# software-mansion/smelter

Measured on AMD Instinct MI355X. Metric: composited frames/sec, 8x1080p->1 4K scene, higher is better.
Workload: dtype u8 (f32 colour conversion: the WGSL sequence value for value; Lanczos on f16-pair MFMA with f32 accumulate, f16 resampler intermediate); 1 GPU; configs[2]: 8x1080p YUV420 inputs tiled -> 3840x2160 YUV420, Tiles + Rescaler(border_radius 24) + text label per tile, GpuOptimized (linear-light Lanczos3 + blend); inputs=8, layouts=33, prime_frames=4676, input_ring=12, frames_in_flight=2, parallelism=single GPU

## Files before the change

### smelter_amd/csrc/smr_fused.hip

```cpp
#include "smr_fused_compose.h"
#include "smr_fused_ingest.h"
#include "smr_ingest_wave.h"

#include <cstdlib>

namespace {

bool fused_disabled(smr_ctx *ctx) {
#ifdef SMR_LAB
    if (!ctx->ablate_read) {
        const char *a = getenv("SMR_ABLATE");
        ctx->ablate = a ? atoi(a) : 0;
        ctx->ablate_read = true;
    }
#endif
    return ctx->fused_disabled == 1;
}

bool frame_is_opaque(u32 fmt) { return frame_format_is_opaque_ycbcr(fmt); }

constexpr size_t SLOT_TARGET = SMR_SLOT_TARGET, SLOT_INGEST_NODE = SMR_SLOT_INGEST_NODE, SLOT_NODE0 = SMR_SLOT_NODE0, SLOT_TILE0 = SMR_SLOT_TILE0,
                 SLOT_TRANSPOSED0 = SMR_SLOT_TRANSPOSED0, SLOT_TRANSPOSED_SINGLE = SMR_SLOT_TRANSPOSED_SINGLE, SLOT_REDUCED0 = SMR_SLOT_REDUCED0;

bool rgb12_node_serves(smr_ctx *ctx, const smr_frame *f, const smr_resample_plan &plan, const smr_surface *tile) {
// ... 485 lines not shown
    }
    if (!wjobs_f16_alpha.empty()) {
        rc = launch_wave(ctx, wjobs_f16_alpha, nullptr, true, true, false, true);
        if (rc != SMR_OK) return rc;
    }
    if (!wjobs_sa_rgba_alpha.empty()) {
        rc = launch_wave(ctx, wjobs_sa_rgba_alpha, nullptr, true, false, true, true);
        if (rc != SMR_OK) return rc;
    }
    if (!wjobs_sa.empty()) {
        rc = launch_wave(ctx, wjobs_sa, nullptr, false, false, true);
        if (rc != SMR_OK) return rc;
    }
    if (!wjobs_sa_rgba.empty()) {
        rc = launch_wave(ctx, wjobs_sa_rgba, nullptr, true, false, true);
        if (rc != SMR_OK) return rc;
    }
    for (const MTransposeBack &b : transposed) {
        rc = launch_transpose<u32>(ctx, b.tile_t, b.tile);
        if (rc != SMR_OK) return rc;
    }
    if (!jobs.empty()) {
        rc = launch_ingest(ctx, jobs);
        if (rc != SMR_OK) return rc;
    }

    if (fuse_out) {
        StageScope scope(ctx, SMR_STAGE_FUSED_COMPOSE);
        ctx->kernel_launches[SMR_KERNEL_COMPOSE_OUTPUT]++;
        u32 n_banded = cm->count_known ? *cm->h_count : n_first * (u32)B_AREA_BANDS;
        if (n_banded > b_tiles * (u32)B_AREA_BANDS) n_banded = b_tiles * (u32)B_AREA_BANDS;
        if (ctx->debug_ingest)
            fprintf(stderr, "k_compose_output: %u tiles, %u bands on the list (%s; predicted tiles %u, last read back %u)\n", b_tiles, n_banded, cm->count_known ? "known" : "predicted", n_first, *cm->h_count);
        dim3 grid(n_banded + (b_tiles + B_COPY_TILES - 1) / B_COPY_TILES, 1, 1);
        const TileList *full = (const TileList *)cm->d_list;
        const TileClass *tc = (const TileClass *)cm->d_class;
        const int flags = (ctx->srgb() ? 1 : 0) | ((ctx->ablate >> 8) << 8);
        SurfView p0, p1, p2;
        int nv;
        if (fuse_rgba) {
            p0 = p1 = p2 = view_of(rgba_target);
            nv = 2;
        } else {
            p0 = view_of(out->planes[0]); p1 = view_of(out->planes[1]);
            nv = out->format == SMR_FRAME_NV12 ? 1 : 0;
            p2 = nv ? p1 : view_of(out->planes[2]);
        }
        typedef void (*ComposeKernel)(SurfView, SurfView, SurfView, int, int, const DevLayout *, const DevMask *, int, int, int, const float *, int, int,
                                      const TileClass *, const TileList *, int, int);
        static const ComposeKernel kernels[3][2] = {{k_compose_output<0, false>, k_compose_output<0, true>},
                                                    {k_compose_output<1, false>, k_compose_output<1, true>},
                                                    {k_compose_output<2, false>, k_compose_output<2, true>}};
        hipLaunchKernelGGL(kernels[nv][big_list ? 1 : 0], grid, dim3(256), 0, ctx->stream, p0, p1, p2, (int)out_w, (int)out_h, packed.layouts, packed.masks,
                           packed.n, packed.n_masks, flags, ctx->d_tables, (int)b_tiles_x, (int)b_tiles, tc, full, (int)n_banded, cm->counter);
        SMR_HIP(ctx, hipGetLastError());
        rc = smr_pack_done(ctx, &packed);
        if (rc != SMR_OK) return rc;
        if (fuse_rgba && out) return smr_rgba_to_frame(ctx, rgba_target, out);
        return SMR_OK;
    }

    smr_surface *target = out_rgba ? out_rgba : smr_cached_surface(ctx, SLOT_TARGET, out_w, out_h, SMR_PX_RGBA8);
    if (!target) return SMR_ERR_OOM;
    rc = smr_launch_apply_layouts(ctx, target, &packed);
    if (rc != SMR_OK) return rc;
    rc = smr_pack_done(ctx, &packed);
    if (rc != SMR_OK) return rc;
// ... 201 lines not shown
```

### smelter_amd/csrc/smr_fused_compose.h

```cpp
#pragma once

#include <type_traits>

#include "smr_convert_dev.h"
#include "smr_layout_dev.h"

namespace {

__device__ __forceinline__ u32 b_off(int row, u32 pitch, int col_bytes) { return (u32)__umul24((u32)row, pitch) + (u32)col_bytes; }

constexpr int B_TILE_W = 128, B_TILE_H = 16;
constexpr int B_MAX_LAYOUTS = 48;
constexpr int B_MAX_MASKS = 96;
static_assert(sizeof(DevLayout) % 16 == 0 && sizeof(DevMask) % 16 == 0, "LDS copies move 16 B words");

#ifndef SMR_COMPOSE_MIN_WAVES
#define SMR_COMPOSE_MIN_WAVES 6
#endif
constexpr int B_MIN_WAVES = SMR_COMPOSE_MIN_WAVES;
constexpr int B_BAND_ROWS = SMR_COMPOSE_BAND_ROWS;
static_assert(B_TILE_H % B_BAND_ROWS == 0 && B_BAND_ROWS >= 2, "a band fits the LDS pixel state");

inline u32 compose_predict(const PackedLayouts &p, int tiles_x, int tiles_y, std::vector<u32> &bitmap) {
    const int tiles = tiles_x * tiles_y, words = (tiles + 31) / 32;
    bitmap.assign((size_t)words, 0u);
    auto mark = [&](float x0, float y0, float x1, float y1) {
        int tx0 = (int)floorf(x0 / (float)B_TILE_W), tx1 = (int)floorf(x1 / (float)B_TILE_W);
        int ty0 = (int)floorf(y0 / (float)B_TILE_H), ty1 = (int)floorf(y1 / (float)B_TILE_H);
        tx0 = tx0 < 0 ? 0 : tx0; ty0 = ty0 < 0 ? 0 : ty0;
        tx1 = tx1 >= tiles_x ? tiles_x - 1 : tx1; ty1 = ty1 >= tiles_y ? tiles_y - 1 : ty1;
        for (int ty = ty0; ty <= ty1; ty++)
            for (int tx = tx0; tx <= tx1; tx++) {
                const int t = ty * tiles_x + tx;
                bitmap[t >> 5] |= 1u << (t & 31);
            }
    };
    auto corners = [&](float left, float top, float w, float h, float c, const DevLayout &L) {
        if (!(c > 0.0f)) return;
        const float bx0 = (float)L.bx0, by0 = (float)L.by0, bx1 = (float)L.bx1 - 1.0f, by1 = (float)L.by1 - 1.0f;
        const float xs[2][2] = {{left, left + c}, {left + w - c, left + w}}, ys[2][2] = {{top, top + c}, {top + h - c, top + h}};
// ... 209 lines not shown
    o.w = div_cr((float)a, 255.0f, 1.0f / 255.0f);
    return o;
}

__device__ __forceinline__ u32 aligned_texel(const DevLayout &L, int px, int py) {
    return g_ld_u32(L.src.ptr + b_off(clampi(py - L.iy, 0, L.tex_h - 1), L.src.pitch, clampi(px - L.ix, 0, L.tex_w - 1) * 4));
}

__device__ __forceinline__ u32 compose_px(u32 a, const DevLayout &L, const DevMask *__restrict__ masks, int px, int py, bool is_base,
                                          u32 raw_pre, int srgb, const float *__restrict__ dec, const float *__restrict__ thr) {
    float fx, fy, lx, ly;
    if (!layout_covers(L, px, py, fx, fy, lx, ly)) return a;
    const bool solid = is_base || layout_solid_box(L, masks, fx, fy, fx, fy);
    if (L.type != 0) {
        if (solid && (L.flags & DL_COLOR_OPAQUE)) return L.solid_px;
        const float4 frag = solid ? make_float4(L.color[0], L.color[1], L.color[2], L.color[3])
                                  : layout_fragment(L, masks, fx, fy, lx, ly, make_float4(0.f, 0.f, 0.f, 0.f));
        return blend_store(a, frag, srgb, dec, thr);
    }
    const bool aligned = (L.flags & DL_ALIGNED) && L.src_kind != 0;
    u32 raw = 0u;
    float4 sample;
    if (aligned) {
        raw = raw_pre;
        sample = decode_texel(raw, srgb, dec);
    } else {
        sample = layout_texture_sample(L, px, py, lx, ly, srgb, dec);
    }
    const float4 frag = solid ? sample : layout_fragment(L, masks, fx, fy, lx, ly, sample);
    if (aligned && (raw >> 24) == 255u && frag.x == sample.x && frag.y == sample.y && frag.z == sample.z && frag.w == sample.w) return raw;
    return blend_store(a, frag, srgb, dec, thr);
}

template <int NV>
__device__ __forceinline__ void store_yuv_block(const u32 (&acc)[8], int px0, int py0, int W, const SurfView &yp, const SurfView &up, const SurfView &vp) {
    const bool half = px0 + 3 >= W;
    if (NV == 2) {
        u8 *o = yp.ptr + b_off(py0, yp.pitch, px0 * 4);
        if (half) {
            *(uint2 *)o = make_uint2(acc[0], acc[1]);
            *(uint2 *)(o + yp.pitch) = make_uint2(acc[4], acc[5]);
        } else {
            *(uint4 *)o = make_uint4(acc[0], acc[1], acc[2], acc[3]);
            *(uint4 *)(o + yp.pitch) = make_uint4(acc[4], acc[5], acc[6], acc[7]);
        }
        return;
    }
    float cr[8], cg[8], cb[8];
#pragma unroll
    for (int k = 0; k < 8; k++) {
        cr[k] = (float)(acc[k] & 0xffu);
        cg[k] = (float)((acc[k] >> 8) & 0xffu);
        cb[k] = (float)((acc[k] >> 16) & 0xffu);
    }
    u32 yrow0 = 0, yrow1 = 0;
#pragma unroll
    for (int k = 0; k < 4; k++) {
        yrow0 |= yuv_luma_byte(acc[k], cr[k], cg[k], cb[k]) << (8 * k);
        yrow1 |= yuv_luma_byte(acc[4 + k], cr[4 + k], cg[4 + k], cb[4 + k]) << (8 * k);
    }
    if (half) {
        *(u16 *)(yp.ptr + b_off(py0, yp.pitch, px0)) = (u16)yrow0;
        *(u16 *)(yp.ptr + b_off(py0 + 1, yp.pitch, px0)) = (u16)yrow1;
    } else {
        *(u32 *)(yp.ptr + b_off(py0, yp.pitch, px0)) = yrow0;
        *(u32 *)(yp.ptr + b_off(py0 + 1, yp.pitch, px0)) = yrow1;
    }
    u32 uv[2][2];
#pragma unroll
    for (int j = 0; j < 2; j++) {
        const int a = 2 * j, b = 2 * j + 1, c = 4 + 2 * j, d = 4 + 2 * j + 1;
        const u32 q = yuv_chroma_bytes(acc[a], acc[b], acc[c], acc[d], (cr[a] + cr[b]) + (cr[c] + cr[d]), (cg[a] + cg[b]) + (cg[c] + cg[d]),
                                       (cb[a] + cb[b]) + (cb[c] + cb[d]));
        uv[j][0] = q & 0xffu;
        uv[j][1] = q >> 8;
    }
    const int cx = px0 >> 1, cy = py0 >> 1;
    if (NV == 0) {
        if (half) {
            up.ptr[b_off(cy, up.pitch, cx)] = (u8)uv[0][0];
            vp.ptr[b_off(cy, vp.pitch, cx)] = (u8)uv[0][1];
        } else {
            *(u16 *)(up.ptr + b_off(cy, up.pitch, cx)) = (u16)(uv[0][0] | (uv[1][0] << 8));
            *(u16 *)(vp.ptr + b_off(cy, vp.pitch, cx)) = (u16)(uv[0][1] | (uv[1][1] << 8));
        }
    } else if (half) {
        *(u16 *)(up.ptr + b_off(cy, up.pitch, cx * 2)) = (u16)(uv[0][0] | (uv[0][1] << 8));
    } else {
        *(u32 *)(up.ptr + b_off(cy, up.pitch, cx * 2)) = uv[0][0] | (uv[0][1] << 8) | (uv[1][0] << 16) | (uv[1][1] << 24);
    }
}

__device__ __forceinline__ u32 list_slot(u32 *count, bool want) {
#ifdef SMR_EMU
    return want ? atomicAdd(count, 1u) : 0u;
#else
    const unsigned long long m = __ballot(want);
    if (m == 0ull) return 0u;
    const u32 rank = __builtin_amdgcn_mbcnt_hi((u32)(m >> 32), __builtin_amdgcn_mbcnt_lo((u32)m, 0u));
    u32 base = 0u;
    if (want && rank == 0u) base = atomicAdd(count, (u32)__popcll(m));
    return (u32)__builtin_amdgcn_readlane((int)base, (int)__builtin_ctzll(m)) + rank;
#endif
}
__device__ __forceinline__ bool wave_any(bool v) {
#ifdef SMR_EMU
    return true;
#else
    return __ballot(v) != 0ull;
#endif
}

template <int NV, bool BIG>
__device__ __forceinline__ void compose_full(const TileFull *__restrict__ pre, int band, int rh, const SurfView &yp, const SurfView &up, const SurfView &vp, int W, int H,
                                             const DevLayout *__restrict__ layouts_g, const DevMask *__restrict__ masks_g, int n, int n_masks,
                                             int srgb_and_ablate, const float *__restrict__ tables, int tiles_x, float *s_tab) {
    const int tile = (int)pre->tile;
    constexpr int BAND_PX = B_TILE_W * B_BAND_ROWS;
    constexpr int SWEEPS = 2;
    static_assert(BAND_PX % 512 == 0 && BAND_PX <= 2048, "whole slabs; a list entry keeps the pixel's index in IDX_BITS bits");
    constexpr int IDX_BITS = BIG ? 11 : (BAND_PX <= 1024 ? 10 : 11);
    constexpr bool WIDE = BIG || ((B_MAX_LAYOUTS + 1) > (1 << (16 - IDX_BITS)));
    typedef typename std::conditional<WIDE, u32, u16>::type entry_t;
    __shared__ u32 s_touch[MAX_LAYOUT_WORDS];
    __shared__ u32 s_px[BAND_PX];
    __shared__ entry_t s_list[BAND_PX];
    __shared__ u32 s_count;
    __shared__ __attribute__((aligned(16))) DevLayout s_lay[B_MAX_LAYOUTS];
    __shared__ __attribute__((aligned(16))) DevMask s_mask[B_MAX_MASKS];
    const int tid = threadIdx.x;
    u32 acc[8] = {0u, 0u, 0u, 0u, 0u, 0u, 0u, 0u};
    const int tile_y = tile / tiles_x;
    const int tx0 = (tile - tile_y * tiles_x) * B_TILE_W, ty0 = tile_y * B_TILE_H + band;
    const int px0 = tx0 + 4 * (tid & 31), py0 = ty0 + 2 * (tid >> 5);
    __syncthreads();
    {
        static_assert(SMR_TABLE_FLOATS % 4 == 0 && SMR_TABLE_FLOATS / 4 <= 256, "one 16 B word of the tables per thread");
        constexpr int LW = (B_MAX_LAYOUTS * (int)(sizeof(DevLayout) / 16) + 255) / 256, MW = (B_MAX_MASKS * (int)(sizeof(DevMask) / 16) + 255) / 256;
        const uint4 *gl = (const uint4 *)layouts_g, *gm = (const uint4 *)masks_g, *gt = (const uint4 *)tables;
        const int nl = BIG ? 0 : n * (int)(sizeof(DevLayout) / 16), nm = BIG ? 0 : n_masks * (int)(sizeof(DevMask) / 16);
        uint4 wl[LW], wm[MW], wt = make_uint4(0u, 0u, 0u, 0u);
#pragma unroll
        for (int k = 0; k < LW; k++) {
            wl[k] = wt;
            if (tid + 256 * k < nl) wl[k] = gl[tid + 256 * k];
        }
#pragma unroll
        for (int k = 0; k < MW; k++) {
            wm[k] = wt;
            if (tid + 256 * k < nm) wm[k] = gm[tid + 256 * k];
        }
        if (tid < SMR_TABLE_FLOATS / 4) wt = gt[tid];
        u32 touch_w = 0u;
        if (tid < MAX_LAYOUT_WORDS) touch_w = pre->touch[tid];
#pragma unroll
        for (int k = 0; k < LW; k++)
            if (tid + 256 * k < nl) ((uint4 *)s_lay)[tid + 256 * k] = wl[k];
#pragma unroll
        for (int k = 0; k < MW; k++)
            if (tid + 256 * k < nm) ((uint4 *)s_mask)[tid + 256 * k] = wm[k];
        if (tid < SMR_TABLE_FLOATS / 4) ((uint4 *)s_tab)[tid] = wt;
        if (tid < MAX_LAYOUT_WORDS) s_touch[tid] = touch_w;
        if (tid == 0) s_count = 0u;
// ... 107 lines not shown
    }
    }
    __syncthreads();

    const u32 total = s_count;
#pragma unroll 1
    for (u32 k0 = 0; k0 < total; k0 += 256u) {
        const bool act = k0 + (u32)tid < total;
        const u32 e = act ? (u32)s_list[k0 + tid] : 0u;
        const int idx = (int)(e & ((1u << IDX_BITS) - 1u)), from = (int)(e >> IDX_BITS) - 1;
        const int px = tx0 + (idx & (B_TILE_W - 1)), py = ty0 + (idx >> 7);
        u32 a = s_px[idx];
        for (int wi = start < 0 ? 0 : (start >> 5); wi < words; wi++) {
            u32 bits = __builtin_amdgcn_readfirstlane(s_touch[wi]);
            if (start >= 0 && wi == (start >> 5)) bits &= ~((2u << (start & 31)) - 1u);
            while (bits) {
                const int li = (wi << 5) + __builtin_ctz(bits);
                bits &= bits - 1;
                const DevLayout *Lp = &layouts[li];
                const int bx0 = __builtin_amdgcn_readfirstlane(Lp->bx0), bx1 = __builtin_amdgcn_readfirstlane(Lp->bx1);
                const int by0 = __builtin_amdgcn_readfirstlane(Lp->by0), by1 = __builtin_amdgcn_readfirstlane(Lp->by1);
                const bool need = act && li > from && px >= bx0 && px < bx1 && py >= by0 && py < by1;
                if (!wave_any(need)) continue;
                const DevLayout L = load_uniform(Lp);
                u32 raw = 0u;
                if (need && L.type == 0 && (L.flags & DL_ALIGNED) && L.src_kind != 0) raw = aligned_texel(L, px, py);
                if (need) a = compose_px(a, L, masks, px, py, false, raw, srgb, dec, thr);
            }
        }
        if (act) s_px[idx] = a;
    }
    __syncthreads();
    if (!no_block) {
        const int lx0 = px0 - tx0, ly0 = py0 - ty0;
        const uint4 t0 = *(const uint4 *)&s_px[ly0 * B_TILE_W + lx0], t1 = *(const uint4 *)&s_px[(ly0 + 1) * B_TILE_W + lx0];
        acc[0] = t0.x; acc[1] = t0.y; acc[2] = t0.z; acc[3] = t0.w;
        acc[4] = t1.x; acc[5] = t1.y; acc[6] = t1.z; acc[7] = t1.w;
        store_yuv_block<NV>(acc, px0, py0, W, yp, up, vp);
    }
}

#ifndef SMR_COPY_TILES
#define SMR_COPY_TILES 1
#endif
constexpr int B_COPY_TILES = SMR_COPY_TILES;
static_assert(B_COPY_TILES == 1 || B_COPY_TILES == 2, "one or two tiles per workgroup");

template <int NV, bool BIG>
__global__ __launch_bounds__(256, B_MIN_WAVES) void k_compose_output(SurfView yp, SurfView up, SurfView vp, int W, int H,
                                                        const DevLayout *__restrict__ layouts_g, const DevMask *__restrict__ masks_g,
                                                        int n, int n_masks, int srgb_and_ablate, const float *__restrict__ tables,
                                                        int tiles_x, int tiles, const TileClass *__restrict__ tc, const TileList *__restrict__ full,
                                                        int n_banded, int counter) {
    const int tid = threadIdx.x;
#if defined(SMR_PRIO_COMPOSE) && !defined(SMR_EMU)
    __builtin_amdgcn_s_setprio(SMR_PRIO_COMPOSE);
#endif
    __shared__ __attribute__((aligned(16))) float s_tab[SMR_TABLE_FLOATS];
    const int rest = (int)blockIdx.x - n_banded;
    const TileFull *full_entry = nullptr, *full_entry2 = nullptr;
    int full_entries = 1, full_entries2 = 1;
    if (rest < 0) {
        if (blockIdx.x >= full->count[counter]) return;
        full_entry = &full->e[blockIdx.x];
    } else {
    const int t0 = rest * B_COPY_TILES;
    const int bx = 4 * (tid & 31), by = 2 * (tid >> 5);
    TileClass c[B_COPY_TILES];
#pragma unroll
    for (int k = 0; k < B_COPY_TILES; k++) {
        c[k] = tc[min(t0 + k, tiles - 1)];
        if (t0 + k >= tiles) c[k].kind = TC_SKIP;
    }
    u32 acc[B_COPY_TILES][8];
    bool on[B_COPY_TILES];
    bool aligned = true;
#pragma unroll
    for (int k = 0; k < B_COPY_TILES; k++) {
        const int tile = t0 + k, ty = tile / tiles_x;
        on[k] = c[k].kind <= TC_TEXTURE && !((srgb_and_ablate >> 8) & 64) && (tile - ty * tiles_x) * B_TILE_W + bx < W && ty * B_TILE_H + by < H;
        if (c[k].kind == TC_TEXTURE && ((((uintptr_t)c[k].base) & 15) != 0 || (c[k].pitch_or_px & 15) != 0)) aligned = false;
        if ((W & 3) && (tile - ty * tiles_x) * B_TILE_W + B_TILE_W > W) aligned = false;
    }
    if (aligned) {
        uint4 ra[B_COPY_TILES], rb[B_COPY_TILES];
#pragma unroll
        for (int k = 0; k < B_COPY_TILES; k++) {
            const bool tex = on[k] && c[k].kind == TC_TEXTURE;
            const u8 *r0 = tex ? c[k].base + b_off(by, c[k].pitch_or_px, bx * 4) : (const u8 *)tables;
            const u8 *r1 = tex ? r0 + c[k].pitch_or_px : (const u8 *)tables;
            ra[k] = g_ld_u32x4(r0);
            rb[k] = g_ld_u32x4(r1);
        }
#pragma unroll
        for (int k = 0; k < B_COPY_TILES; k++) {
            const bool tex = c[k].kind == TC_TEXTURE;
            const u32 fill = c[k].kind == TC_COLOUR ? c[k].pitch_or_px : 0u;
            acc[k][0] = tex ? ra[k].x : fill; acc[k][1] = tex ? ra[k].y : fill; acc[k][2] = tex ? ra[k].z : fill; acc[k][3] = tex ? ra[k].w : fill;
            acc[k][4] = tex ? rb[k].x : fill; acc[k][5] = tex ? rb[k].y : fill; acc[k][6] = tex ? rb[k].z : fill; acc[k][7] = tex ? rb[k].w : fill;
        }
    } else {
#pragma unroll
        for (int k = 0; k < B_COPY_TILES; k++) {
            const u32 fill = c[k].kind == TC_COLOUR ? c[k].pitch_or_px : 0u;
#pragma unroll
            for (int q = 0; q < 8; q++) acc[k][q] = fill;
            if (on[k] && c[k].kind == TC_TEXTURE) {
                const u8 *r0 = c[k].base + b_off(by, c[k].pitch_or_px, bx * 4), *r1 = r0 + c[k].pitch_or_px;
                const int tile = t0 + k, cols = W - ((tile - (tile / tiles_x) * tiles_x) * B_TILE_W + bx);
#pragma unroll
                for (int q = 0; q < 4; q++)
                    if (q < cols) { acc[k][q] = g_ld_u32(r0 + 4 * q); acc[k][4 + q] = g_ld_u32(r1 + 4 * q); }
            }
        }
    }
#pragma unroll
    for (int k = 0; k < B_COPY_TILES; k++) {
        const int tile = t0 + k, ty = tile / tiles_x;
        if (on[k]) store_yuv_block<NV>(acc[k], (tile - ty * tiles_x) * B_TILE_W + bx, ty * B_TILE_H + by, W, yp, up, vp);
    }
#pragma unroll 1
    for (int k = 0; k < B_COPY_TILES; k++) {
        if (c[k].kind != TC_SAMPLED || ((srgb_and_ablate >> 8) & 32)) continue;
        __syncthreads();
        for (int i = tid; i < SMR_TABLE_FLOATS; i += 256) s_tab[i] = tables[i];
        __syncthreads();
        const DevLayout L = load_uniform(&layouts_g[c[k].pitch_or_px]);
        const int tile = t0 + k, ty = tile / tiles_x;
        const int px0 = (tile - ty * tiles_x) * B_TILE_W + bx, py0 = ty * B_TILE_H + by;
        if (px0 < W && py0 < H) {
            u32 a[8];
            composite_sampled_opaque_block(L, px0, py0, srgb_and_ablate & 1, s_tab, s_tab + 256, a);
            store_yuv_block<NV>(a, px0, py0, W, yp, up, vp);
        }
    }
#pragma unroll 1
    for (int k = 0; k < B_COPY_TILES; k++) {
        if (c[k].kind != TC_SELECT) continue;
        const int tile = t0 + k, ty = tile / tiles_x;
        const int px0 = (tile - ty * tiles_x) * B_TILE_W + bx, py0 = ty * B_TILE_H + by;
        u32 a[8] = {0u, 0u, 0u, 0u, 0u, 0u, 0u, 0u};
        u32 open_px = 0xffu;
#pragma unroll 1
        for (int q = 0; q < 4; q++) {
            const u32 li = (c[k].pitch_or_px >> (8 * q)) & 0xffu;
            if (li == 0xffu) break;
            const DevLayout &L = layouts_g[li];
            const int lx0 = L.bx0, ly0 = L.by0, lx1 = L.bx1, ly1 = L.by1;
            const bool colour = L.type != 0;
            const u32 solid = L.solid_px;
#pragma unroll
            for (int i = 0; i < 8; i++) {
                const int px = px0 + (i & 3), py = py0 + (i >> 2);
                if (((open_px >> i) & 1u) && px >= lx0 && px < lx1 && py >= ly0 && py < ly1) {
                    a[i] = colour ? solid : aligned_texel(L, px, py);
                    open_px &= ~(1u << i);
                }
            }
        }
        if (px0 < W && py0 < H) store_yuv_block<NV>(a, px0, py0, W, yp, up, vp);
    }
    if (c[0].kind == TC_FULL && (int)c[0].pitch_or_px + (int)(uintptr_t)c[0].base > n_banded) {
        full_entry = &full->e[c[0].pitch_or_px];
        full_entries = (int)(uintptr_t)c[0].base;
    }
    if (B_COPY_TILES > 1 && c[B_COPY_TILES - 1].kind == TC_FULL && (int)c[B_COPY_TILES - 1].pitch_or_px + (int)(uintptr_t)c[B_COPY_TILES - 1].base > n_banded) {
        const TileFull *e = &full->e[c[B_COPY_TILES - 1].pitch_or_px];
        if (full_entry) { full_entry2 = e; full_entries2 = (int)(uintptr_t)c[B_COPY_TILES - 1].base; }
        else { full_entry = e; full_entries = (int)(uintptr_t)c[B_COPY_TILES - 1].base; }
    }
    }
#ifdef SMR_COMPOSE_NO_FULL
    if (full_entry || full_entry2) return;
#endif
#pragma unroll 1
    for (int q = 0; q < 2; q++) {
        const TileFull *e = q == 0 ? full_entry : full_entry2;
        if (!e) break;
        const int entries = q == 0 ? full_entries : full_entries2;
#pragma unroll 1
        for (int j = 0; j < entries; j++) {
            if (rest >= 0 && (int)(e - full->e) + j < n_banded) continue;
            const u32 bw = __builtin_amdgcn_readfirstlane(e[j].band);
            compose_full<NV, BIG>(&e[j], (int)(bw & 0xffu), (int)(bw >> 8), yp, up, vp, W, H, layouts_g, masks_g, n, n_masks, srgb_and_ablate, tables, tiles_x, s_tab);
        }
    }
}

}
```

### smelter_amd/csrc/smr_ingest_common.h

```cpp
#pragma once

#include "smr_convert_dev.h"
#include "smr_resample_dev.h"

typedef _Float16 f16x8 __attribute__((ext_vector_type(8)));
typedef float f32x4 __attribute__((ext_vector_type(4)));

#ifdef SMR_EMU
#include "emu_device.h"
#else
#define dev_perm(hi, lo, sel) __builtin_amdgcn_perm((hi), (lo), (sel))
#define dev_alignbyte(hi, lo, sh) __builtin_amdgcn_alignbyte((hi), (lo), (sh))
#define dev_udot4(a, b, c) __builtin_amdgcn_udot4((a), (b), (c), false)
#define dev_fmed3(a, b, c) __builtin_amdgcn_fmed3f((a), (b), (c))
#define dev_mad24(a, b, c) ((u32)__umul24((a), (b)) + (c))
#define dev_readfirstlane(x) __builtin_amdgcn_readfirstlane(x)
#define dev_mfma_16x16x32_f16(a, b, c) __builtin_amdgcn_mfma_f32_16x16x32_f16((a), (b), (c), 0, 0, 0)
#define dev_wait_vmcnt0() __builtin_amdgcn_s_waitcnt(0x0f70)
#define dev_mov_dpp_quad_swap(x) __builtin_amdgcn_mov_dpp((x), 0xb1, 0xf, 0xf, true)
#define dev_sched_barrier() __builtin_amdgcn_sched_barrier(0)
#define dev_wave_lds_sync() __builtin_amdgcn_wave_barrier()
__device__ __forceinline__ u32 dev_lds_u32(u32 byte_offset) {
    typedef __attribute__((address_space(3))) const u32 lds_u32;
    return *(lds_u32 *)(uintptr_t)byte_offset;
}
#endif

namespace {

struct MConv {
    float ky, krv, kgu, kgv, kbu, cr, cg, cb, ylo, yhi, clo, chi;
};

constexpr int M_LUT_ENTRIES = 768;

struct MDirect {
    const u8 *cls;
    int tiles_x, nv;
    SurfView yp, up, vp;
};

inline MConv m_conv_constants(bool full) {
    const double ys = full ? 1.0 : 255.0 / 219.0, y0 = full ? 0.0 : 16.0;
    const double cs = full ? 1.0 / 16.0 : 255.0 / (16.0 * 224.0);
    const double c0 = full ? 0.0 : 16.0 * 16.0, half = full ? 16.0 * 127.5 : 16.0 * 112.0;
    MConv K;
    K.ky = (float)ys;
    K.krv = (float)(1.5748 * cs); K.kgu = (float)(-0.1873 * cs); K.kgv = (float)(-0.4681 * cs); K.kbu = (float)(1.8556 * cs);
    const double bias = 1024.0 + 256.0 + 0.5;
    K.cr = (float)(bias - ys * y0 - 1.5748 * cs * (c0 + half));
    K.cg = (float)(bias - ys * y0 + (0.1873 + 0.4681) * cs * (c0 + half));
    K.cb = (float)(bias - ys * y0 - 1.8556 * cs * (c0 + half));
// ... 79 lines not shown
```

### smelter_amd/csrc/smr_internal.h

```cpp
#pragma once


#include <hip/hip_runtime.h>
#include <hip/hip_fp16.h>

#include <cstdarg>
#include <cstdint>
#include <cstdio>
#include <cstring>
#include <string>
#include <vector>

#include "smr.h"

constexpr int SMR_INGEST_LAB_FUSED = 5;
#ifdef SMR_LAB
constexpr bool SMR_LAB_BUILD = true;
#else
constexpr bool SMR_LAB_BUILD = false;
#endif

#ifndef SMR_COMPOSE_BAND_ROWS
#define SMR_COMPOSE_BAND_ROWS 8
#endif
// ... 5 lines not shown
#define SMR_ENC_ENTRIES 1664
#define SMR_LUT16_WORDS (256 + SMR_ENC_ENTRIES)

#define SMR_NUM_STAGES 8
enum {
    SMR_STAGE_INGEST = 0,
    SMR_STAGE_RESAMPLE = 1,
    SMR_STAGE_LAYOUT = 2,
    SMR_STAGE_OUTPUT = 3,
    SMR_STAGE_FUSED_INGEST = 4,
    SMR_STAGE_FUSED_COMPOSE = 5,
};

constexpr size_t SMR_SURFACE_TAIL = 16;

struct smr_surface {
    void *ptr = nullptr;
    size_t pitch = 0;
    u32 w = 0, h = 0, fmt = 0;
    bool owned = false;
    size_t capacity = 0;

};

#if defined(__HIPCC__) && !defined(SMR_EMU)
typedef u32 g_u32x2 __attribute__((ext_vector_type(2)));
typedef u32 g_u32x3 __attribute__((ext_vector_type(3)));
typedef u32 g_u32x4 __attribute__((ext_vector_type(4)));
#define SMR_GLOBAL_PTR(T, p) ((__attribute__((address_space(1))) T *)(uintptr_t)(p))
__device__ __forceinline__ u32 g_ld_u32(const void *p) { return *SMR_GLOBAL_PTR(const u32, p); }
__device__ __forceinline__ uint2 g_ld_u32x2(const void *p) { const g_u32x2 v = *SMR_GLOBAL_PTR(const g_u32x2, p); return make_uint2(v.x, v.y); }
__device__ __forceinline__ uint4 g_ld_u32x4(const void *p) { const g_u32x4 v = *SMR_GLOBAL_PTR(const g_u32x4, p); return make_uint4(v.x, v.y, v.z, v.w); }
__device__ __forceinline__ void g_st_u32(void *p, u32 v) { *SMR_GLOBAL_PTR(u32, p) = v; }
__device__ __forceinline__ void g_st_u32x3(void *p, u32 a, u32 b, u32 c) { g_u32x3 v; v.x = a; v.y = b; v.z = c; *SMR_GLOBAL_PTR(g_u32x3, p) = v; }
__device__ __forceinline__ void g_st_u32x4(void *p, uint4 q) { g_u32x4 v; v.x = q.x; v.y = q.y; v.z = q.z; v.w = q.w; *SMR_GLOBAL_PTR(g_u32x4, p) = v; }
typedef int g_i32x2 __attribute__((ext_vector_type(2)));
__device__ __forceinline__ int2 g_ld_uniform_i32x2(const void *p) { const g_i32x2 v = *((__attribute__((address_space(4))) const g_i32x2 *)(uintptr_t)(p)); return make_int2(v.x, v.y); }
#define SMR_KEEP_SCALAR(x) asm volatile("" : "+s"(x))
#else
static inline u32 g_ld_u32(const void *p) { return *(const u32 *)p; }
static inline uint2 g_ld_u32x2(const void *p) { return *(const uint2 *)p; }
static inline uint4 g_ld_u32x4(const void *p) { return *(const uint4 *)p; }
static inline void g_st_u32(void *p, u32 v) { *(u32 *)p = v; }
static inline void g_st_u32x3(void *p, u32 a, u32 b, u32 c) { ((u32 *)p)[0] = a; ((u32 *)p)[1] = b; ((u32 *)p)[2] = c; }
static inline void g_st_u32x4(void *p, uint4 q) { *(uint4 *)p = q; }
static inline int2 g_ld_uniform_i32x2(const void *p) { return *(const int2 *)p; }
#define SMR_KEEP_SCALAR(x) do { } while (0)
#endif

struct LayoutSlot {
    void *host = nullptr;
    void *dev = nullptr;
    size_t bytes = 0;
    hipEvent_t done = nullptr;
    bool busy = false;
    bool unfenced = false;
    size_t resident_bytes = 0;
    uint64_t last_reuse = 0;
};

struct StagePending {
    hipEvent_t a, b;
    int stage;
};

struct TileClassMap {
    std::vector<uint8_t> key;
    bool ready = false;
    void *d_class = nullptr;
    uint8_t *d_direct = nullptr;
    void *d_list = nullptr;
    size_t n = 0;
    uint32_t *h_count = nullptr;
    hipEvent_t count_ev = nullptr;
    bool count_pending = false, count_known = false;
    uint64_t class_serial = 0, count_serial = 0;
// ... 188 lines not shown
```

Before: 19900 frames/s.

## Pair YUV stores across lanes, fast colour path with repair, multi-tile copy runs

Converts RGB to YUV with a fast yuvfast path and recomputes exactly only when a flag marks a byte as uncertain. Adjacent lanes trade rows and chroma through DPP quad swaps, so each lane issues one wider 8-byte luma store and one 4-byte chroma store instead of several narrow ones. Copy workgroups now walk a short run of tiles, prefetching the next tile's texels while storing the current one, which halves the copy grid. The cost is more per-lane control flow, an extra branch on the repair path, and a deferred pass for sampled, select and full tiles.

```diff
diff --git a/smelter_amd/csrc/smr_fused.hip b/smelter_amd/csrc/smr_fused.hip
--- a/smelter_amd/csrc/smr_fused.hip
+++ b/smelter_amd/csrc/smr_fused.hip
@@ -541,7 +541,7 @@
         if (n_banded > b_tiles * (u32)B_AREA_BANDS) n_banded = b_tiles * (u32)B_AREA_BANDS;
         if (ctx->debug_ingest)
             fprintf(stderr, "k_compose_output: %u tiles, %u bands on the list (%s; predicted tiles %u, last read back %u)\n", b_tiles, n_banded, cm->count_known ? "known" : "predicted", n_first, *cm->h_count);
-        dim3 grid(n_banded + (b_tiles + B_COPY_TILES - 1) / B_COPY_TILES, 1, 1);
+        dim3 grid(n_banded + (b_tiles + B_COPY_RUN - 1) / B_COPY_RUN, 1, 1);
         const TileList *full = (const TileList *)cm->d_list;
         const TileClass *tc = (const TileClass *)cm->d_class;
         const int flags = (ctx->srgb() ? 1 : 0) | ((ctx->ablate >> 8) << 8);
diff --git a/smelter_amd/csrc/smr_fused_compose.h b/smelter_amd/csrc/smr_fused_compose.h
--- a/smelter_amd/csrc/smr_fused_compose.h
+++ b/smelter_amd/csrc/smr_fused_compose.h
@@ -6,6 +6,12 @@
 #include "smr_layout_dev.h"
 
 namespace {
+
+#ifdef SMR_EMU
+#define B_KEEP_IN_LOOP(x) do { } while (0)
+#else
+#define B_KEEP_IN_LOOP(x) asm volatile("" : "+v"(x))
+#endif
 
 __device__ __forceinline__ u32 b_off(int row, u32 pitch, int col_bytes) { return (u32)__umul24((u32)row, pitch) + (u32)col_bytes; }
 
@@ -281,8 +287,59 @@
     return blend_store(a, frag, srgb, dec, thr);
 }
 
+__device__ __forceinline__ void yuv_block_repair(const u32 (&acc)[8], u32 &yrow0, u32 &yrow1, u32 &u2, u32 &v2) {
+    u32 px[8];
+    float r[8], g[8], b[8];
+#pragma unroll
+    for (int k = 0; k < 8; k++) {
+        px[k] = acc[k];
+        B_KEEP_IN_LOOP(px[k]);
+        r[k] = unorm_of_byte(px[k] & 0xffu);
+        g[k] = unorm_of_byte((px[k] >> 8) & 0xffu);
+        b[k] = unorm_of_byte((px[k] >> 16) & 0xffu);
+    }
+#pragma unroll
+    for (int k = 0; k < 8; k++) {
+        bool f;
+        (void)yuvfast::convert<0>((float)(px[k] & 0xffu), (float)((px[k] >> 8) & 0xffu), (float)((px[k] >> 16) & 0xffu), &f);
+        const u32 exact = yuv_byte(r[k], g[k], b[k], 0), sh = 8u * (u32)(k & 3);
+        u32 &row = k < 4 ? yrow0 : yrow1;
+        row = f ? ((row & ~(0xffu << sh)) | (exact << sh)) : row;
+    }
+#pragma unroll
+    for (int j = 0; j < 2; j++) {
+        const int a = 2 * j, c = 4 + 2 * j;
+        float sum[3];
+#pragma unroll
+        for (int ch = 0; ch < 3; ch++)
+            sum[ch] = ((float)((px[a] >> (8 * ch)) & 0xffu) + (float)((px[a + 1] >> (8 * ch)) & 0xffu)) +
+                      ((float)((px[c] >> (8 * ch)) & 0xffu) + (float)((px[c + 1] >> (8 * ch)) & 0xffu));
+        bool f1, f2;
+        (void)yuvfast::convert<1>(sum[0], sum[1], sum[2], &f1);
+        (void)yuvfast::convert<2>(sum[0], sum[1], sum[2], &f2);
+        const float mr = ((r[a] + r[a + 1]) + (r[c] + r[c + 1])) * 0.25f, mg = ((g[a] + g[a + 1]) + (g[c] + g[c + 1])) * 0.25f,
+                    mb = ((b[a] + b[a + 1]) + (b[c] + b[c + 1])) * 0.25f;
+        const u32 eu = yuv_byte(mr, mg, mb, 1), ev = yuv_byte(mr, mg, mb, 2), sh = 8u * (u32)j;
+        u2 = f1 ? ((u2 & ~(0xffu << sh)) | (eu << sh)) : u2;
+        v2 = f2 ? ((v2 & ~(0xffu << sh)) | (ev << sh)) : v2;
+    }
+}
+
 template <int NV>
-__device__ __forceinline__ void store_yuv_block(const u32 (&acc)[8], int px0, int py0, int W, const SurfView &yp, const SurfView &up, const SurfView &vp) {
+__device__ __forceinline__ bool planes_pair_aligned(const SurfView &yp, const SurfView &up, const SurfView &vp) {
+#if defined(SMR_EMU) && !defined(SMR_EMU_WAVE_EXCHANGE)
+    return false;
+#else
+    if (NV == 2) return false;
+    bool ok = ((((uintptr_t)yp.ptr) | yp.pitch) & 7u) == 0;
+    if (NV == 0) ok = ok && ((((uintptr_t)up.ptr) | up.pitch | ((uintptr_t)vp.ptr) | vp.pitch) & 3u) == 0;
+    return ok;
+#endif
+}
+
+template <int NV>
+__device__ __forceinline__ void store_yuv_block(const u32 (&acc)[8], int px0, int py0, int W, const SurfView &yp, const SurfView &up, const SurfView &vp,
+                                                bool pair = false) {
     const bool half = px0 + 3 >= W;
     if (NV == 2) {
         u8 *o = yp.ptr + b_off(py0, yp.pitch, px0 * 4);
@@ -302,11 +359,42 @@
         cg[k] = (float)((acc[k] >> 8) & 0xffu);
         cb[k] = (float)((acc[k] >> 16) & 0xffu);
     }
-    u32 yrow0 = 0, yrow1 = 0;
+    u32 yrow0 = 0, yrow1 = 0, u2 = 0, v2 = 0;
+    bool flagged = false;
 #pragma unroll
     for (int k = 0; k < 4; k++) {
-        yrow0 |= yuv_luma_byte(acc[k], cr[k], cg[k], cb[k]) << (8 * k);
-        yrow1 |= yuv_luma_byte(acc[4 + k], cr[4 + k], cg[4 + k], cb[4 + k]) << (8 * k);
+        bool f0, f1;
+        yrow0 |= yuvfast::convert<0>(cr[k], cg[k], cb[k], &f0) << (8 * k);
+        yrow1 |= yuvfast::convert<0>(cr[4 + k], cg[4 + k], cb[4 + k], &f1) << (8 * k);
+        flagged |= f0 | f1;
+    }
+#pragma unroll
+    for (int j = 0; j < 2; j++) {
+        const int a = 2 * j, b = 2 * j + 1, c = 4 + 2 * j, d = 4 + 2 * j + 1;
+        const float sr = (cr[a] + cr[b]) + (cr[c] + cr[d]), sg = (cg[a] + cg[b]) + (cg[c] + cg[d]), sb = (cb[a] + cb[b]) + (cb[c] + cb[d]);
+        bool f1, f2;
+        u2 |= yuvfast::convert<1>(sr, sg, sb, &f1) << (8 * j);
+        v2 |= yuvfast::convert<2>(sr, sg, sb, &f2) << (8 * j);
+        flagged |= f1 | f2;
+    }
+    if (flagged) {
+        YUV_SLOW_PATH_STAYS_A_BRANCH();
+        yuv_block_repair(acc, yrow0, yrow1, u2, v2);
+    }
+    const u32 uv4 = (u2 & 0xffu) | ((v2 & 0xffu) << 8) | ((u2 & 0xff00u) << 8) | ((v2 & 0xff00u) << 16);
+    const int cx = px0 >> 1, cy = py0 >> 1;
+    if (pair) {
+        const bool odd = (px0 & 4) != 0;
+        const u32 ny = (u32)dev_mov_dpp_quad_swap((int)(odd ? yrow0 : yrow1));
+        g_st_u32x2(yp.ptr + b_off(py0 + (odd ? 1 : 0), yp.pitch, px0 & ~7), odd ? ny : yrow0, odd ? yrow1 : ny);
+        if (NV == 0) {
+            const u32 nc = (u32)dev_mov_dpp_quad_swap((int)(odd ? u2 : v2));
+            u8 *o = odd ? vp.ptr + b_off(cy, vp.pitch, cx & ~3) : up.ptr + b_off(cy, up.pitch, cx);
+            g_st_u32(o, odd ? (nc | (v2 << 16)) : (u2 | (nc << 16)));
+        } else {
+            *(u32 *)(up.ptr + b_off(cy, up.pitch, cx * 2)) = uv4;
+        }
+        return;
     }
     if (half) {
         *(u16 *)(yp.ptr + b_off(py0, yp.pitch, px0)) = (u16)yrow0;
@@ -315,28 +403,18 @@
         *(u32 *)(yp.ptr + b_off(py0, yp.pitch, px0)) = yrow0;
         *(u32 *)(yp.ptr + b_off(py0 + 1, yp.pitch, px0)) = yrow1;
     }
-    u32 uv[2][2];
-#pragma unroll
-    for (int j = 0; j < 2; j++) {
-        const int a = 2 * j, b = 2 * j + 1, c = 4 + 2 * j, d = 4 + 2 * j + 1;
-        const u32 q = yuv_chroma_bytes(acc[a], acc[b], acc[c], acc[d], (cr[a] + cr[b]) + (cr[c] + cr[d]), (cg[a] + cg[b]) + (cg[c] + cg[d]),
-                                       (cb[a] + cb[b]) + (cb[c] + cb[d]));
-        uv[j][0] = q & 0xffu;
-        uv[j][1] = q >> 8;
-    }
-    const int cx = px0 >> 1, cy = py0 >> 1;
     if (NV == 0) {
         if (half) {
-            up.ptr[b_off(cy, up.pitch, cx)] = (u8)uv[0][0];
-            vp.ptr[b_off(cy, vp.pitch, cx)] = (u8)uv[0][1];
+            up.ptr[b_off(cy, up.pitch, cx)] = (u8)u2;
+            vp.ptr[b_off(cy, vp.pitch, cx)] = (u8)v2;
         } else {
-            *(u16 *)(up.ptr + b_off(cy, up.pitch, cx)) = (u16)(uv[0][0] | (uv[1][0] << 8));
-            *(u16 *)(vp.ptr + b_off(cy, vp.pitch, cx)) = (u16)(uv[0][1] | (uv[1][1] << 8));
+            *(u16 *)(up.ptr + b_off(cy, up.pitch, cx)) = (u16)u2;
+            *(u16 *)(vp.ptr + b_off(cy, vp.pitch, cx)) = (u16)v2;
         }
     } else if (half) {
-        *(u16 *)(up.ptr + b_off(cy, up.pitch, cx * 2)) = (u16)(uv[0][0] | (uv[0][1] << 8));
+        *(u16 *)(up.ptr + b_off(cy, up.pitch, cx * 2)) = (u16)uv4;
     } else {
-        *(u32 *)(up.ptr + b_off(cy, up.pitch, cx * 2)) = uv[0][0] | (uv[0][1] << 8) | (uv[1][0] << 16) | (uv[1][1] << 24);
+        *(u32 *)(up.ptr + b_off(cy, up.pitch, cx * 2)) = uv4;
     }
 }
 
@@ -377,7 +455,9 @@
     __shared__ u32 s_count;
     __shared__ __attribute__((aligned(16))) DevLayout s_lay[B_MAX_LAYOUTS];
     __shared__ __attribute__((aligned(16))) DevMask s_mask[B_MAX_MASKS];
-    const int tid = threadIdx.x;
+    int tid = threadIdx.x;
+    B_KEEP_IN_LOOP(tid);
+    tid &= 255;
     u32 acc[8] = {0u, 0u, 0u, 0u, 0u, 0u, 0u, 0u};
     const int tile_y = tile / tiles_x;
     const int tx0 = (tile - tile_y * tiles_x) * B_TILE_W, ty0 = tile_y * B_TILE_H + band;
@@ -551,19 +631,43 @@
     }
     __syncthreads();
     if (!no_block) {
-        const int lx0 = px0 - tx0, ly0 = py0 - ty0;
+        int ltid = tid;
+        B_KEEP_IN_LOOP(ltid);
+        const int lx0 = 4 * (ltid & 31), ly0 = 2 * (ltid >> 5), px0 = tx0 + lx0, py0 = ty0 + ly0;
         const uint4 t0 = *(const uint4 *)&s_px[ly0 * B_TILE_W + lx0], t1 = *(const uint4 *)&s_px[(ly0 + 1) * B_TILE_W + lx0];
         acc[0] = t0.x; acc[1] = t0.y; acc[2] = t0.z; acc[3] = t0.w;
         acc[4] = t1.x; acc[5] = t1.y; acc[6] = t1.z; acc[7] = t1.w;
-        store_yuv_block<NV>(acc, px0, py0, W, yp, up, vp);
-    }
-}
-
-#ifndef SMR_COPY_TILES
-#define SMR_COPY_TILES 1
+        const bool pair = tx0 + B_TILE_W <= W && tile_y * B_TILE_H + B_TILE_H <= H && (rh & 3) == 0 && planes_pair_aligned<NV>(yp, up, vp);
+        store_yuv_block<NV>(acc, px0, py0, W, yp, up, vp, pair);
+    }
+}
+
+constexpr int B_COPY_TILES = 1;
+#ifndef SMR_COPY_RUN
+#define SMR_COPY_RUN 2
 #endif
-constexpr int B_COPY_TILES = SMR_COPY_TILES;
-static_assert(B_COPY_TILES == 1 || B_COPY_TILES == 2, "one or two tiles per workgroup");
+constexpr int B_COPY_RUN = SMR_COPY_RUN;
+static_assert(B_COPY_RUN >= 1 && B_COPY_RUN <= 4, "a short run: the grid stays larger than what is resident");
+
+__device__ __forceinline__ void copy_tile_texels(const TileClass &c, bool on, int cols, int bx, int by, const float *__restrict__ tables, u32 (&t)[8]) {
+    const u32 fill = c.kind == TC_COLOUR ? c.pitch_or_px : 0u;
+#pragma unroll
+    for (int q = 0; q < 8; q++) t[q] = fill;
+    if (c.kind != TC_TEXTURE) return;
+    const bool aligned = ((((uintptr_t)c.base) | c.pitch_or_px) & 15) == 0 && !((cols & 3) != 0 && cols < B_TILE_W);
+    if (aligned) {
+        const u8 *r0 = on ? c.base + b_off(by, c.pitch_or_px, bx * 4) : (const u8 *)tables;
+        const u8 *r1 = on ? r0 + c.pitch_or_px : (const u8 *)tables;
+        const uint4 ra = g_ld_u32x4(r0), rb = g_ld_u32x4(r1);
+        t[0] = ra.x; t[1] = ra.y; t[2] = ra.z; t[3] = ra.w;
+        t[4] = rb.x; t[5] = rb.y; t[6] = rb.z; t[7] = rb.w;
+    } else if (on) {
+        const u8 *r0 = c.base + b_off(by, c.pitch_or_px, bx * 4), *r1 = r0 + c.pitch_or_px;
+#pragma unroll
+        for (int q = 0; q < 4; q++)
+            if (bx + q < cols) { t[q] = g_ld_u32(r0 + 4 * q); t[4 + q] = g_ld_u32(r1 + 4 * q); }
+    }
+}
 
 template <int NV, bool BIG>
 __global__ __launch_bounds__(256, B_MIN_WAVES) void k_compose_output(SurfView yp, SurfView up, SurfView vp, int W, int H,
@@ -577,133 +681,122 @@
 #endif
     __shared__ __attribute__((aligned(16))) float s_tab[SMR_TABLE_FLOATS];
     const int rest = (int)blockIdx.x - n_banded;
-    const TileFull *full_entry = nullptr, *full_entry2 = nullptr;
-    int full_entries = 1, full_entries2 = 1;
+    int t_begin = 0, t_end = 0;
+    bool later = false, left_out = false;
     if (rest < 0) {
         if (blockIdx.x >= full->count[counter]) return;
-        full_entry = &full->e[blockIdx.x];
     } else {
-    const int t0 = rest * B_COPY_TILES;
-    const int bx = 4 * (tid & 31), by = 2 * (tid >> 5);
-    TileClass c[B_COPY_TILES];
-#pragma unroll
-    for (int k = 0; k < B_COPY_TILES; k++) {
-        c[k] = tc[min(t0 + k, tiles - 1)];
-        if (t0 + k >= tiles) c[k].kind = TC_SKIP;
-    }
-    u32 acc[B_COPY_TILES][8];
-    bool on[B_COPY_TILES];
-    bool aligned = true;
-#pragma unroll
-    for (int k = 0; k < B_COPY_TILES; k++) {
-        const int tile = t0 + k, ty = tile / tiles_x;
-        on[k] = c[k].kind <= TC_TEXTURE && !((srgb_and_ablate >> 8) & 64) && (tile - ty * tiles_x) * B_TILE_W + bx < W && ty * B_TILE_H + by < H;
-        if (c[k].kind == TC_TEXTURE && ((((uintptr_t)c[k].base) & 15) != 0 || (c[k].pitch_or_px & 15) != 0)) aligned = false;
-        if ((W & 3) && (tile - ty * tiles_x) * B_TILE_W + B_TILE_W > W) aligned = false;
-    }
-    if (aligned) {
-        uint4 ra[B_COPY_TILES], rb[B_COPY_TILES];
-#pragma unroll
-        for (int k = 0; k < B_COPY_TILES; k++) {
-            const bool tex = on[k] && c[k].kind == TC_TEXTURE;
-            const u8 *r0 = tex ? c[k].base + b_off(by, c[k].pitch_or_px, bx * 4) : (const u8 *)tables;
-            const u8 *r1 = tex ? r0 + c[k].pitch_or_px : (const u8 *)tables;
-            ra[k] = g_ld_u32x4(r0);
-            rb[k] = g_ld_u32x4(r1);
-        }
-#pragma unroll
-        for (int k = 0; k < B_COPY_TILES; k++) {
-            const bool tex = c[k].kind == TC_TEXTURE;
-            const u32 fill = c[k].kind == TC_COLOUR ? c[k].pitch_or_px : 0u;
-            acc[k][0] = tex ? ra[k].x : fill; acc[k][1] = tex ? ra[k].y : fill; acc[k][2] = tex ? ra[k].z : fill; acc[k][3] = tex ? ra[k].w : fill;
-            acc[k][4] = tex ? rb[k].x : fill; acc[k][5] = tex ? rb[k].y : fill; acc[k][6] = tex ? rb[k].z : fill; acc[k][7] = tex ? rb[k].w : fill;
-        }
-    } else {
-#pragma unroll
-        for (int k = 0; k < B_COPY_TILES; k++) {
-            const u32 fill = c[k].kind == TC_COLOUR ? c[k].pitch_or_px : 0u;
-#pragma unroll
-            for (int q = 0; q < 8; q++) acc[k][q] = fill;
-            if (on[k] && c[k].kind == TC_TEXTURE) {
-                const u8 *r0 = c[k].base + b_off(by, c[k].pitch_or_px, bx * 4), *r1 = r0 + c[k].pitch_or_px;
-                const int tile = t0 + k, cols = W - ((tile - (tile / tiles_x) * tiles_x) * B_TILE_W + bx);
-#pragma unroll
-                for (int q = 0; q < 4; q++)
-                    if (q < cols) { acc[k][q] = g_ld_u32(r0 + 4 * q); acc[k][4 + q] = g_ld_u32(r1 + 4 * q); }
-            }
-        }
-    }
-#pragma unroll
-    for (int k = 0; k < B_COPY_TILES; k++) {
-        const int tile = t0 + k, ty = tile / tiles_x;
-        if (on[k]) store_yuv_block<NV>(acc[k], (tile - ty * tiles_x) * B_TILE_W + bx, ty * B_TILE_H + by, W, yp, up, vp);
-    }
+        const int groups = (int)gridDim.x - n_banded;
+        const int run = (tiles + groups - 1) / groups;
+        t_begin = rest * run;
+        t_end = min(t_begin + run, tiles);
+        if (t_begin >= t_end) return;
+        const bool ablate_copy = ((srgb_and_ablate >> 8) & 64) != 0;
+        const bool planes_ok = planes_pair_aligned<NV>(yp, up, vp);
+        int t = t_begin;
+        const int ty = t / tiles_x;
+        int tx0 = (t - ty * tiles_x) * B_TILE_W, ty0 = ty * B_TILE_H;
+        TileClass c0 = tc[t], c1 = tc[min(t + 1, tiles - 1)], c2;
+        u32 cur[8];
+        copy_tile_texels(c0, tx0 + 4 * (tid & 31) < W && ty0 + 2 * (tid >> 5) < H && !ablate_copy, W - tx0, 4 * (tid & 31), 2 * (tid >> 5), tables, cur);
 #pragma unroll 1
-    for (int k = 0; k < B_COPY_TILES; k++) {
-        if (c[k].kind != TC_SAMPLED || ((srgb_and_ablate >> 8) & 32)) continue;
-        __syncthreads();
-        for (int i = tid; i < SMR_TABLE_FLOATS; i += 256) s_tab[i] = tables[i];
-        __syncthreads();
-        const DevLayout L = load_uniform(&layouts_g[c[k].pitch_or_px]);
-        const int tile = t0 + k, ty = tile / tiles_x;
-        const int px0 = (tile - ty * tiles_x) * B_TILE_W + bx, py0 = ty * B_TILE_H + by;
-        if (px0 < W && py0 < H) {
-            u32 a[8];
-            composite_sampled_opaque_block(L, px0, py0, srgb_and_ablate & 1, s_tab, s_tab + 256, a);
-            store_yuv_block<NV>(a, px0, py0, W, yp, up, vp);
-        }
-    }
+        for (;;) {
+            int ltid = tid;
+            B_KEEP_IN_LOOP(ltid);
+            const int bx = 4 * (ltid & 31), by = 2 * (ltid >> 5);
+            const int px0 = tx0 + bx, py0 = ty0 + by;
+            const bool inside = px0 < W && py0 < H;
+            const bool pair = planes_ok && tx0 + B_TILE_W <= W && ty0 + B_TILE_H <= H;
+            c2 = tc[min(t + 2, tiles - 1)];
+            u32 nxt[8] = {0u, 0u, 0u, 0u, 0u, 0u, 0u, 0u};
+            const bool wrap = tx0 + B_TILE_W >= tiles_x * B_TILE_W;
+            const int nx0 = wrap ? 0 : tx0 + B_TILE_W, ny0 = wrap ? ty0 + B_TILE_H : ty0;
+            if (t + 1 < t_end) copy_tile_texels(c1, nx0 + bx < W && ny0 + by < H && !ablate_copy, W - nx0, bx, by, tables, nxt);
+            if (c0.kind <= TC_TEXTURE) {
+                if (inside && !ablate_copy) store_yuv_block<NV>(cur, px0, py0, W, yp, up, vp, pair);
+            } else if (c0.kind == TC_SAMPLED || c0.kind == TC_SELECT) {
+                later = true;
+            } else if (c0.kind == TC_FULL && (int)c0.pitch_or_px + (int)(uintptr_t)c0.base > n_banded) {
+                left_out = true;
+            }
+            if (++t >= t_end) break;
+#pragma unroll
+            for (int q = 0; q < 8; q++) cur[q] = nxt[q];
+            c0 = c1; c1 = c2;
+            tx0 = nx0; ty0 = ny0;
+        }
+        if (!later && !left_out) return;
+    }
+    if (later) {
 #pragma unroll 1
-    for (int k = 0; k < B_COPY_TILES; k++) {
-        if (c[k].kind != TC_SELECT) continue;
-        const int tile = t0 + k, ty = tile / tiles_x;
-        const int px0 = (tile - ty * tiles_x) * B_TILE_W + bx, py0 = ty * B_TILE_H + by;
-        u32 a[8] = {0u, 0u, 0u, 0u, 0u, 0u, 0u, 0u};
-        u32 open_px = 0xffu;
+        for (int t = t_begin; t < t_end; t++) {
+            const TileClass c = tc[t];
+            if (c.kind != TC_SAMPLED && c.kind != TC_SELECT) continue;
+            int ltid = tid;
+            B_KEEP_IN_LOOP(ltid);
+            const int ty = t / tiles_x, tx0 = (t - ty * tiles_x) * B_TILE_W, ty0 = ty * B_TILE_H;
+            const int px0 = tx0 + 4 * (ltid & 31), py0 = ty0 + 2 * (ltid >> 5);
+            const bool inside = px0 < W && py0 < H;
+            const bool pair = tx0 + B_TILE_W <= W && ty0 + B_TILE_H <= H && planes_pair_aligned<NV>(yp, up, vp);
+            if (c.kind == TC_SAMPLED) {
+                if ((srgb_and_ablate >> 8) & 32) continue;
+                __syncthreads();
+                for (int i = ltid; i < SMR_TABLE_FLOATS; i += 256) s_tab[i] = tables[i];
+                __syncthreads();
+                const DevLayout L = load_uniform(&layouts_g[c.pitch_or_px]);
+                if (inside) {
+                    u32 a[8];
+                    composite_sampled_opaque_block(L, px0, py0, srgb_and_ablate & 1, s_tab, s_tab + 256, a);
+                    store_yuv_block<NV>(a, px0, py0, W, yp, up, vp, pair);
+                }
+            } else if (c.kind == TC_SELECT) {
+                u32 a[8] = {0u, 0u, 0u, 0u, 0u, 0u, 0u, 0u};
+                u32 open_px = 0xffu;
 #pragma unroll 1
-        for (int q = 0; q < 4; q++) {
-            const u32 li = (c[k].pitch_or_px >> (8 * q)) & 0xffu;
-            if (li == 0xffu) break;
-            const DevLayout &L = layouts_g[li];
-            const int lx0 = L.bx0, ly0 = L.by0, lx1 = L.bx1, ly1 = L.by1;
-            const bool colour = L.type != 0;
-            const u32 solid = L.solid_px;
-#pragma unroll
-            for (int i = 0; i < 8; i++) {
-                const int px = px0 + (i & 3), py = py0 + (i >> 2);
-                if (((open_px >> i) & 1u) && px >= lx0 && px < lx1 && py >= ly0 && py < ly1) {
-                    a[i] = colour ? solid : aligned_texel(L, px, py);
-                    open_px &= ~(1u << i);
+                for (int q = 0; q < 4; q++) {
+                    const u32 li = (c.pitch_or_px >> (8 * q)) & 0xffu;
+                    if (li == 0xffu) break;
+                    const DevLayout &L = layouts_g[li];
+                    const int lx0 = L.bx0, ly0 = L.by0, lx1 = L.bx1, ly1 = L.by1;
+                    const bool colour = L.type != 0;
+                    const u32 solid = L.solid_px;
+#pragma unroll
+                    for (int i = 0; i < 8; i++) {
+                        const int px = px0 + (i & 3), py = py0 + (i >> 2);
+                        if (((open_px >> i) & 1u) && px >= lx0 && px < lx1 && py >= ly0 && py < ly1) {
+                            a[i] = colour ? solid : aligned_texel(L, px, py);
+                            open_px &= ~(1u << i);
+                        }
+                    }
                 }
-            }
-        }
-        if (px0 < W && py0 < H) store_yuv_block<NV>(a, px0, py0, W, yp, up, vp);
-    }
-    if (c[0].kind == TC_FULL && (int)c[0].pitch_or_px + (int)(uintptr_t)c[0].base > n_banded) {
-        full_entry = &full->e[c[0].pitch_or_px];
-        full_entries = (int)(uintptr_t)c[0].base;
-    }
-    if (B_COPY_TILES > 1 && c[B_COPY_TILES - 1].kind == TC_FULL && (int)c[B_COPY_TILES - 1].pitch_or_px + (int)(uintptr_t)c[B_COPY_TILES - 1].base > n_banded) {
-        const TileFull *e = &full->e[c[B_COPY_TILES - 1].pitch_or_px];
-        if (full_entry) { full_entry2 = e; full_entries2 = (int)(uintptr_t)c[B_COPY_TILES - 1].base; }
-        else { full_entry = e; full_entries = (int)(uintptr_t)c[B_COPY_TILES - 1].base; }
-    }
-    }
-#ifdef SMR_COMPOSE_NO_FULL
-    if (full_entry || full_entry2) return;
-#endif
+                if (inside) store_yuv_block<NV>(a, px0, py0, W, yp, up, vp, pair);
+            }
+        }
+        if (!left_out) return;
+    }
 #pragma unroll 1
-    for (int q = 0; q < 2; q++) {
-        const TileFull *e = q == 0 ? full_entry : full_entry2;
-        if (!e) break;
-        const int entries = q == 0 ? full_entries : full_entries2;
+    for (int t = t_begin;; t++) {
+        const TileFull *e;
+        int entries = 1;
+        if (rest < 0) {
+            e = &full->e[blockIdx.x];
+        } else {
+            if (t >= t_end) break;
+            const TileClass c = tc[t];
+            if (!(c.kind == TC_FULL && (int)c.pitch_or_px + (int)(uintptr_t)c.base > n_banded)) continue;
+            e = &full->e[c.pitch_or_px];
+            entries = (int)(uintptr_t)c.base;
+        }
+#ifndef SMR_COMPOSE_NO_FULL
 #pragma unroll 1
         for (int j = 0; j < entries; j++) {
             if (rest >= 0 && (int)(e - full->e) + j < n_banded) continue;
             const u32 bw = __builtin_amdgcn_readfirstlane(e[j].band);
             compose_full<NV, BIG>(&e[j], (int)(bw & 0xffu), (int)(bw >> 8), yp, up, vp, W, H, layouts_g, masks_g, n, n_masks, srgb_and_ablate, tables, tiles_x, s_tab);
         }
-    }
-}
-
-}
+#endif
+        if (rest < 0) break;
+    }
+}
+
+}
diff --git a/smelter_amd/csrc/smr_ingest_common.h b/smelter_amd/csrc/smr_ingest_common.h
--- a/smelter_amd/csrc/smr_ingest_common.h
+++ b/smelter_amd/csrc/smr_ingest_common.h
@@ -17,7 +17,6 @@
 #define dev_readfirstlane(x) __builtin_amdgcn_readfirstlane(x)
 #define dev_mfma_16x16x32_f16(a, b, c) __builtin_amdgcn_mfma_f32_16x16x32_f16((a), (b), (c), 0, 0, 0)
 #define dev_wait_vmcnt0() __builtin_amdgcn_s_waitcnt(0x0f70)
-#define dev_mov_dpp_quad_swap(x) __builtin_amdgcn_mov_dpp((x), 0xb1, 0xf, 0xf, true)
 #define dev_sched_barrier() __builtin_amdgcn_sched_barrier(0)
 #define dev_wave_lds_sync() __builtin_amdgcn_wave_barrier()
 __device__ __forceinline__ u32 dev_lds_u32(u32 byte_offset) {
diff --git a/smelter_amd/csrc/smr_internal.h b/smelter_amd/csrc/smr_internal.h
--- a/smelter_amd/csrc/smr_internal.h
+++ b/smelter_amd/csrc/smr_internal.h
@@ -61,16 +61,19 @@
 __device__ __forceinline__ uint2 g_ld_u32x2(const void *p) { const g_u32x2 v = *SMR_GLOBAL_PTR(const g_u32x2, p); return make_uint2(v.x, v.y); }
 __device__ __forceinline__ uint4 g_ld_u32x4(const void *p) { const g_u32x4 v = *SMR_GLOBAL_PTR(const g_u32x4, p); return make_uint4(v.x, v.y, v.z, v.w); }
 __device__ __forceinline__ void g_st_u32(void *p, u32 v) { *SMR_GLOBAL_PTR(u32, p) = v; }
+__device__ __forceinline__ void g_st_u32x2(void *p, u32 a, u32 b) { g_u32x2 v; v.x = a; v.y = b; *SMR_GLOBAL_PTR(g_u32x2, p) = v; }
 __device__ __forceinline__ void g_st_u32x3(void *p, u32 a, u32 b, u32 c) { g_u32x3 v; v.x = a; v.y = b; v.z = c; *SMR_GLOBAL_PTR(g_u32x3, p) = v; }
 __device__ __forceinline__ void g_st_u32x4(void *p, uint4 q) { g_u32x4 v; v.x = q.x; v.y = q.y; v.z = q.z; v.w = q.w; *SMR_GLOBAL_PTR(g_u32x4, p) = v; }
 typedef int g_i32x2 __attribute__((ext_vector_type(2)));
 __device__ __forceinline__ int2 g_ld_uniform_i32x2(const void *p) { const g_i32x2 v = *((__attribute__((address_space(4))) const g_i32x2 *)(uintptr_t)(p)); return make_int2(v.x, v.y); }
 #define SMR_KEEP_SCALAR(x) asm volatile("" : "+s"(x))
+#define dev_mov_dpp_quad_swap(x) __builtin_amdgcn_mov_dpp((x), 0xb1, 0xf, 0xf, true)
 #else
 static inline u32 g_ld_u32(const void *p) { return *(const u32 *)p; }
 static inline uint2 g_ld_u32x2(const void *p) { return *(const uint2 *)p; }
 static inline uint4 g_ld_u32x4(const void *p) { return *(const uint4 *)p; }
 static inline void g_st_u32(void *p, u32 v) { *(u32 *)p = v; }
+static inline void g_st_u32x2(void *p, u32 a, u32 b) { ((u32 *)p)[0] = a; ((u32 *)p)[1] = b; }
 static inline void g_st_u32x3(void *p, u32 a, u32 b, u32 c) { ((u32 *)p)[0] = a; ((u32 *)p)[1] = b; ((u32 *)p)[2] = c; }
 static inline void g_st_u32x4(void *p, uint4 q) { *(uint4 *)p = q; }
 static inline int2 g_ld_uniform_i32x2(const void *p) { return *(const int2 *)p; }
```

Result: faster. 20850 frames/s (median of 6 runs) (+4.8%).
